# saiprasadbarke/robustmvd

Hardware: AMD Instinct MI355X
Metric: depth-maps/sec at 768x1152x4srcx256planes; warp+aggregate HBM GB/s vs roofline (higher is better)
Workload: dtype f32; 1 GPU; mvsnet (Path B) forward 768x1152, 4 source views, 256 planes, batch 1 per step (BASELINE.json configs[2]); the regulariser's two layers with 32 input channels (conv0, conv4): every fp32 operand as two range-scaled fp16 terms on fp16 MFMA, fp32 accumulation (at least as close to a float64 convolution as the fp32 matrix instruction over 1e-42..1e30: tests/test_hip_f16.py), the other nine layers and ; parallelism=1 independent replica(s), frames round-robin, no collectives

## Files before the change

### robustmvd_amd/csrc/conv3d_split.hip

```cpp
#include "mvd_common.h"
#include "split_operand.h"

#ifndef SPLIT_KO
#define SPLIT_KO 0
#endif
#ifndef SPLIT_DEPTH
#define SPLIT_DEPTH 4
#endif

namespace mvd {

typedef _Float16 h16x8 __attribute__((ext_vector_type(8)));
typedef float sf32x4 __attribute__((ext_vector_type(4)));
typedef unsigned int su32x4 __attribute__((ext_vector_type(4)));
typedef unsigned int su32x2 __attribute__((ext_vector_type(2)));
typedef _Float16 h16x2 __attribute__((ext_vector_type(2)));

constexpr int S_TH = 4, S_TW = 32, S_ROWS = S_TH + 2;
constexpr float S_LO_FACTOR = 2048.0f;
template <int CIN>
struct SplitGeom {
    static constexpr int CH8 = CIN / 8;
    static constexpr int VB = CIN * 2;
    static constexpr int KWG = CIN == 32 ? 3 : 2;
    static constexpr int NT = 9 * KWG;
    static constexpr int COLS = CIN == 32 ? S_TW + 2 : S_TW + 3;
    static constexpr int HALF_BYTES = S_ROWS * COLS * VB;
    static constexpr int PLANE_BYTES = 2 * HALF_BYTES;
    static constexpr int ITEMS = S_ROWS * COLS * CH8;
    static constexpr int NLOAD = (ITEMS + 255) / 256;
    static constexpr int NF = 4 * KWG * 2;
    static_assert(NF - 8 == 4 * NLOAD, "pass B interleaves 8 epilogue groups and 4 staging groups per item");
};

template <int CIN>
__global__ void pack_conv0_split_kernel(const float* __restrict__ w, const float* __restrict__ wscale, _Float16* __restrict__ packed, int ncb) {
    using G = SplitGeom<CIN>;
    const int e = blockIdx.x * 256 + threadIdx.x;
    if (e >= ncb * G::NT * 64 * 8) return;
    const int j = e & 7, lane = (e >> 3) & 63, t = (e >> 9) % G::NT, cb = (e >> 9) / G::NT;
    const int col = lane & 15, k = 8 * (lane >> 4) + j, cout = cb * 8 + (col & 7);
    int tap, cin;
    if constexpr (CIN == 32) { tap = t; cin = k; }
    else { const int kw = 2 * (t % 2) + k / 16; tap = kw < 3 ? (t / 2) * 3 + kw : -1; cin = k % 16; }
    const float v = tap >= 0 ? w[((size_t)cout * CIN + cin) * 27 + tap] / wscale[cout] : 0.0f;
    _Float16 hi, lo;
    split_weight(v, S_LO_FACTOR, hi, lo);
    packed[e] = col < 8 ? hi : lo;
}

struct SplitParams {
    const float* x;
    const char* wpk;
    const float* scale;
    const float* shift;
    const float* absmax;
    float* y;
    float* yamax;
    int B, D, h, w, relu;
    int cout, ncb;
    int tiles_x, tiles_y, dgroups, td, tiles_per_xcd;
};

__device__ __forceinline__ unsigned pack_h2(_Float16 a, _Float16 b) {
    const h16x2 v = {a, b};
    return __builtin_bit_cast(unsigned, v);
}

template <int CIN, bool YAMAX = false>
__global__ void __launch_bounds__(256, 2) conv0_split_kernel(SplitParams p) {
    using G = SplitGeom<CIN>;
    constexpr int S_COLS = G::COLS, S_HALF_BYTES = G::HALF_BYTES, S_PLANE_BYTES = G::PLANE_BYTES, S_ITEMS = G::ITEMS, S_NLOAD = G::NLOAD;
    constexpr int KWG = G::KWG, NT = G::NT;
    extern __shared__ __attribute__((aligned(16))) char ring[];
    const int tid = threadIdx.x, lane = tid & 63, wv = tid >> 6;
    const int D = p.D, h = p.h, w = p.w;

    const int xcd = blockIdx.x & 7;
    int j = blockIdx.x >> 3;
    const int cb = j % p.ncb; j /= p.ncb;
    const int t_in = j % p.tiles_per_xcd; j /= p.tiles_per_xcd;
    const int dg = j % p.dgroups;
    const int b = j / p.dgroups;
    const int tile = xcd * p.tiles_per_xcd + t_in;
    if (tile >= p.tiles_x * p.tiles_y) return;
    const int ty = tile / p.tiles_x, tx = tile - ty * p.tiles_x;
    const int x0 = tx * S_TW, y0 = ty * S_TH;
    const int dz0 = dg * p.td, dz1 = min(dz0 + p.td, D);

    h16x8 wf[NT];
#pragma unroll
    for (int t = 0; t < NT; ++t) wf[t] = *reinterpret_cast<const h16x8*>(p.wpk + (((size_t)cb * NT + t) * 64 + lane) * 16);

    constexpr unsigned OOB = 0x80000000u;
    unsigned gob[S_NLOAD];
    int loff[S_NLOAD];
#pragma unroll
    for (int k = 0; k < S_NLOAD; ++k) {
        const int e = tid + 256 * k;
        const int vox = e / G::CH8, ch = e % G::CH8;
        const int r = vox / S_COLS, c = vox - r * S_COLS;
        const int gy = y0 - 1 + r, gx = x0 - 1 + c;
        const bool in = e < S_ITEMS && c < S_TW + 2 && gy >= 0 && gy < h && gx >= 0 && gx < w;
        gob[k] = in ? (unsigned)(((gy * w + gx) * CIN + ch * 8) * 4) : OOB;
        if constexpr (CIN == 32) loff[k] = e < S_ITEMS ? (vox * 64 + ((ch ^ ((c >> 1) & 3)) * 16)) : -1;
        else loff[k] = e < S_ITEMS ? e * 16 : -1;
    }
    const size_t plane_f = (size_t)h * w * CIN;
    const float* xb = p.x + (size_t)b * D * plane_f;
    su32x4 pre[S_NLOAD][2];
    auto fetch = [&](int d) {
        const bool din = d >= 0 && d < D && d <= dz1;
        const __amdgpu_buffer_rsrc_t rs = __builtin_amdgcn_make_buffer_rsrc(
            const_cast<float*>(xb + (din ? (size_t)d * plane_f : 0)), 0, din ? (int)(plane_f * 4) : 0, 0x00020000);
#pragma unroll
        for (int k = 0; k < S_NLOAD; ++k) {
            pre[k][0] = __builtin_amdgcn_raw_buffer_load_b128(rs, gob[k], 0, 0);
            pre[k][1] = __builtin_amdgcn_raw_buffer_load_b128(rs, gob[k] + 16u, 0, 0);
        }
    };
    char* const dump = ring + 2 * S_PLANE_BYTES + tid * 16;
    float xs, xs_inv;
    split_xscale(p.absmax, xs, xs_inv);
    auto split2 = [xs](float a0, float a1, unsigned& hi, unsigned& lo) { mvd::split2(xs, a0, a1, hi, lo, S_LO_FACTOR); };
    auto stash = [&](int d) {
        char* slot = ring + (d & 1) * S_PLANE_BYTES;
#pragma unroll
        for (int k = 0; k < S_NLOAD; ++k) {
            su32x4 hv, lv;
#pragma unroll
            for (int q = 0; q < 4; ++q) {
                const sf32x4 v = __builtin_bit_cast(sf32x4, pre[k][q >> 1]);
                unsigned hi, lo;
                split2(v[(q & 1) * 2], v[(q & 1) * 2 + 1], hi, lo);
                hv[q] = hi; lv[q] = lo;
            }
            char* dst = loff[k] >= 0 ? slot + loff[k] : dump;
            *reinterpret_cast<su32x4*>(dst) = hv;
            *reinterpret_cast<su32x4*>(loff[k] >= 0 ? dst + S_HALF_BYTES : dst) = lv;
        }
    };

    const int col = lane & 15;
    float esc_ = p.scale[cb * 8 + (col & 7)], esh_ = p.shift[cb * 8 + (col & 7)];
    float eun_ = reinterpret_cast<const float*>(p.wpk + (size_t)p.ncb * NT * 64 * 16)[cb * 8 + (col & 7)] * xs_inv;
    const float floor_ = p.relu ? 0.f : -__builtin_inff();
    const int xh = wv & 1, rp = wv >> 1;

    int fragk[KWG];
#pragma unroll
    for (int kw = 0; kw < KWG; ++kw) {
        if constexpr (CIN == 32) {
            const int c = 16 * xh + (lane & 15) + kw;
            fragk[kw] = (2 * rp * S_COLS + c) * 64 + (((lane >> 4) ^ ((c >> 1) & 3)) * 16);
        } else {
            const int c = 16 * xh + (lane & 15) + 2 * kw;
            fragk[kw] = (2 * rp * S_COLS + c) * 32 + (lane >> 4) * 16;
        }
    }

    sf32x4 acc[3][2][2];
#pragma unroll
    for (int s = 0; s < 3; ++s)
#pragma unroll
        for (int r = 0; r < 2; ++r) { acc[s][r][0] = sf32x4{0, 0, 0, 0}; acc[s][r][1] = sf32x4{0, 0, 0, 0}; }

    unsigned yoff[2];
#pragma unroll
    for (int row = 0; row < 2; ++row) {
        const int oy = y0 + 2 * rp + row;
        yoff[row] = (col < 8 && oy < h) ? (unsigned)((((size_t)oy * w + x0 + 16 * xh + 4 * (lane >> 4)) * p.cout + cb * 8 + col) * 4) : OOB;
    }
    const int oxb = x0 + 16 * xh + 4 * (lane >> 4);
    const size_t yplane_f = (size_t)h * w * p.cout;
    const unsigned vox_b = (unsigned)p.cout * 4u;

    fetch(dz0 - 1);
    asm volatile("" : "+v"(esc_), "+v"(esh_), "+v"(eun_));
    stash(dz0 - 1);
    fetch(dz0);

    [[maybe_unused]] float amax_ = 0.f;
    for (int z = dz0 - 1; z <= dz1; ++z) {
        if (!(SPLIT_KO & 8)) __syncthreads();
        const char* slot = ring + (z & 1) * S_PLANE_BYTES;
        char* wslot = ring + ((z + 1) & 1) * S_PLANE_BYTES;
        const int din = z + 2, dout = z - 1;
        const bool in_ok = din >= 0 && din < D && din <= dz1, out_ok = dout >= dz0 && dout < dz1;
        const __amdgpu_buffer_rsrc_t rs_in = __builtin_amdgcn_make_buffer_rsrc(
            const_cast<float*>(xb + (in_ok ? (size_t)din * plane_f : 0)), 0, in_ok ? (int)(plane_f * 4) : 0, 0x00020000);
        const __amdgpu_buffer_rsrc_t rs_out = __builtin_amdgcn_make_buffer_rsrc(
            p.y + ((size_t)b * D + (out_ok ? dout : 0)) * yplane_f, 0, out_ok ? (int)(yplane_f * 4) : 0, 0x00020000);
        int ox = oxb;
        asm volatile("" : "+v"(ox));

        constexpr int NF = G::NF, NR = 2 * NF, DEPTH = SPLIT_DEPTH;
        h16x8 fr[DEPTH];
        auto rr_of = [](int ro) { return ro == 0 ? 1 : ro == 1 ? 2 : ro == 2 ? 0 : 3; };
        auto frag = [&](int i) {
            const int g = i % NF, term = g & 1, kw = (g >> 1) % KWG, rr = rr_of(g / (2 * KWG));
            if (SPLIT_KO & 32) return wf[i % NT];
            return *reinterpret_cast<const h16x8*>(slot + term * S_HALF_BYTES + fragk[kw] + rr * S_COLS * G::VB);
        };
#pragma unroll
        for (int i = 0; i < DEPTH; ++i) fr[i] = frag(i);
#pragma unroll
        for (int g = 0; g < NF; ++g) {
            const int term = g & 1, kw = (g >> 1) % KWG, rr = rr_of(g / (2 * KWG));
            const h16x8 f = fr[g % DEPTH];
#pragma unroll
            for (int row = 0; row < 2; ++row) {
                const int kh = rr - row;
                if (kh < 0 || kh > 2) continue;
                if (SPLIT_KO & 16) acc[0][row][term][0] += f[0] * wf[(6 + kh) * KWG + kw][0];
                else acc[0][row][term] = __builtin_amdgcn_mfma_f32_16x16x32_f16(f, wf[(6 + kh) * KWG + kw], acc[0][row][term], 0, 0, 0);
            }
            fr[g % DEPTH] = frag(g + DEPTH);
            __builtin_amdgcn_sched_barrier(0);
        }
        float hl = __shfl_down(acc[0][0][0][0], 8, 16);
        unsigned hq0 = 0, lq0 = 0;
#pragma unroll
        for (int g = 0; g < NF; ++g) {
            const int term = g & 1, kw = (g >> 1) % KWG, rr = rr_of(g / (2 * KWG));
            const h16x8 f = fr[(NF + g) % DEPTH];
#pragma unroll
            for (int row = 0; row < 2; ++row) {
                const int kh = rr - row;
                if (kh < 0 || kh > 2) continue;
#pragma unroll
                for (int s = 1; s < 3; ++s)
                    if (SPLIT_KO & 16) acc[s][row][term][0] += f[0] * wf[((2 - s) * 3 + kh) * KWG + kw][0];
                    else acc[s][row][term] = __builtin_amdgcn_mfma_f32_16x16x32_f16(f, wf[((2 - s) * 3 + kh) * KWG + kw], acc[s][row][term], 0, 0, 0);
            }
            if (NF + g + DEPTH < NR) fr[(NF + g) % DEPTH] = frag(NF + g + DEPTH);
            if (g < 8) {
                const int row = g >> 2, i = g & 3;
                const float cur = hl;
                if (g + 1 < 8) hl = __shfl_down(acc[0][(g + 1) >> 2][0][(g + 1) & 3], 8, 16);
                float r = __builtin_fmaf(cur + acc[0][row][1][i], 1.0f / 2048.0f, acc[0][row][0][i]);
                r = fmaxf(__builtin_fmaf(r * eun_, esc_, esh_), floor_);
                if constexpr (YAMAX)
                    if (out_ok && yoff[row] != OOB && ox + i < w) amax_ = fmaxf(amax_, finite_abs_or_zero(r));
                if (!(SPLIT_KO & 2) || r == 12345.678f)
                    __builtin_amdgcn_raw_buffer_store_b32(__float_as_uint(r), rs_out, ox + i < w ? yoff[row] + vox_b * i : OOB, 0, 0);
            } else if (!(SPLIT_KO & 4)) {
                const int k = (g - 8) >> 2, q = (g - 8) & 3;
                const sf32x4 v = __builtin_bit_cast(sf32x4, pre[k][q >> 1]);
                unsigned hq1, lq1;
                split2(v[(q & 1) * 2], v[(q & 1) * 2 + 1], hq1, lq1);
                if (q & 1) {
                    char* dst = (loff[k] >= 0 ? wslot + loff[k] : dump) + 8 * (q >> 1);
                    *reinterpret_cast<su32x2*>(dst) = su32x2{hq0, hq1};
                    *reinterpret_cast<su32x2*>(loff[k] >= 0 ? dst + S_HALF_BYTES : dst) = su32x2{lq0, lq1};
                } else {
                    hq0 = hq1; lq0 = lq1;
                }
                if (q == 3 && !(SPLIT_KO & 1)) {
                    pre[k][0] = __builtin_amdgcn_raw_buffer_load_b128(rs_in, gob[k], 0, 0);
                    pre[k][1] = __builtin_amdgcn_raw_buffer_load_b128(rs_in, gob[k] + 16u, 0, 0);
                }
            }
            __builtin_amdgcn_sched_barrier(0);
        }
#pragma unroll
        for (int r = 0; r < 2; ++r)
#pragma unroll
            for (int t = 0; t < 2; ++t) {
                acc[0][r][t] = acc[1][r][t];
                acc[1][r][t] = acc[2][r][t];
                acc[2][r][t] = sf32x4{0, 0, 0, 0};
            }
    }
    if constexpr (YAMAX) {
        for (int o = 32; o > 0; o >>= 1) amax_ = fmaxf(amax_, __shfl_xor(amax_, o));
        __syncthreads();
        float* wm = reinterpret_cast<float*>(ring);
        if (lane == 0) wm[wv] = amax_;
        __syncthreads();
        if (tid == 0) {
            amax_ = fmaxf(fmaxf(wm[0], wm[1]), fmaxf(wm[2], wm[3]));
            raise_absmax(p.yamax, amax_);
        }
    }
}

}

static bool split_shape_ok(int Cin, int Cout) { return (Cin == 32 || Cin == 16) && Cout >= 8 && Cout <= 64 && Cout % 8 == 0; }
static size_t split_frag_bytes(int Cin, int Cout) { return (size_t)(Cout / 8) * (Cin == 32 ? 27 : 18) * 64 * 16; }

template <int CIN, bool YAMAX>
static int launch_split_v(const mvd::SplitParams& p, long long nblk, hipStream_t st) {
    const size_t lds = 2 * (size_t)mvd::SplitGeom<CIN>::PLANE_BYTES + 256 * 16;
    (void)hipFuncSetAttribute((const void*)mvd::conv0_split_kernel<CIN, YAMAX>, hipFuncAttributeMaxDynamicSharedMemorySize, (int)lds);
    hipLaunchKernelGGL((mvd::conv0_split_kernel<CIN, YAMAX>), dim3((unsigned)nblk), dim3(256), lds, st, p);
    return mvd::launch_status("conv3d_split");
}
template <int CIN>
static int launch_split(const mvd::SplitParams& p, long long nblk, hipStream_t st) {
    return p.yamax ? launch_split_v<CIN, true>(p, nblk, st) : launch_split_v<CIN, false>(p, nblk, st);
}

extern "C" {

size_t mvd_conv3d_split_packed_weight_bytes(int Cin, int Cout) {
    return split_shape_ok(Cin, Cout) ? split_frag_bytes(Cin, Cout) + (size_t)Cout * sizeof(float) : 0;
}

int mvd_pack_conv3d_weights_split(const float* w, int Cin, int Cout, void* packed, mvd_stream_t stream) {
    MVD_REQUIRE(w && packed, "pack_conv3d_weights_split: NULL argument");
    MVD_REQUIRE(split_shape_ok(Cin, Cout), "pack_conv3d_weights_split: 16 or 32 input channels and 8, 16, ... 64 output channels are built (got %d -> %d)", Cin, Cout);
    const int ncb = Cout / 8;
    float* wscale = reinterpret_cast<float*>(static_cast<char*>(packed) + split_frag_bytes(Cin, Cout));
    mvd::split_wscale_launch(w, wscale, Cin, Cout, 27, false, Cout, Cout, (hipStream_t)stream);
    const unsigned nb = (unsigned)((split_frag_bytes(Cin, Cout) / 2 + 255) / 256);
    if (Cin == 32) hipLaunchKernelGGL(mvd::pack_conv0_split_kernel<32>, dim3(nb), dim3(256), 0, (hipStream_t)stream, w, wscale, (_Float16*)packed, ncb);
    else hipLaunchKernelGGL(mvd::pack_conv0_split_kernel<16>, dim3(nb), dim3(256), 0, (hipStream_t)stream, w, wscale, (_Float16*)packed, ncb);
    return mvd::launch_status("pack_conv3d_weights_split");
}

static int conv3d_split_entry(const float* x, const float* x_absmax, const void* packed_w, const float* scale, const float* shift, float* y,
                              float* y_absmax, int B, int D, int h, int w, int Cin, int Cout, int relu, mvd_stream_t stream);

int mvd_conv3d_bn_relu_f32_split(const float* x, const float* x_absmax, const void* packed_w, const float* scale, const float* shift,
                                 float* y, int B, int D, int h, int w, int Cin, int Cout, int relu, mvd_stream_t stream) {
    return conv3d_split_entry(x, x_absmax, packed_w, scale, shift, y, nullptr, B, D, h, w, Cin, Cout, relu, stream);
}

int mvd_conv3d_bn_relu_absmax_f32_split(const float* x, const float* x_absmax, const void* packed_w, const float* scale, const float* shift,
                                        float* y, float* y_absmax, int B, int D, int h, int w, int Cin, int Cout, int relu,
                                        mvd_stream_t stream) {
    MVD_REQUIRE(y_absmax, "conv3d_split_absmax: NULL argument");
    return conv3d_split_entry(x, x_absmax, packed_w, scale, shift, y, y_absmax, B, D, h, w, Cin, Cout, relu, stream);
}

static int conv3d_split_entry(const float* x, const float* x_absmax, const void* packed_w, const float* scale, const float* shift, float* y,
                              float* y_absmax, int B, int D, int h, int w, int Cin, int Cout, int relu, mvd_stream_t stream) {
    MVD_REQUIRE(x && x_absmax && packed_w && scale && shift && y, "conv3d_split: NULL argument");
    MVD_REQUIRE(split_shape_ok(Cin, Cout), "conv3d_split: 16 or 32 input channels and 8, 16, ... 64 output channels are built (got %d -> %d)", Cin, Cout);
    MVD_REQUIRE(B > 0 && D > 0 && h > 0 && w > 0, "conv3d_split: non-positive dimension");
    MVD_REQUIRE((long long)h * w * Cin * 4 < 0x7fffffffLL && (long long)h * w * Cout * 4 < 0x7fffffffLL,
                "conv3d_split: one plane exceeds the 31-bit byte-offset range");
    mvd::SplitParams p{};
    p.x = x; p.absmax = x_absmax; p.wpk = (const char*)packed_w; p.scale = scale; p.shift = shift; p.y = y; p.yamax = y_absmax;
    if (y_absmax && hipMemsetAsync(y_absmax, 0, sizeof(float), (hipStream_t)stream) != hipSuccess) return mvd::launch_status("conv3d_split: memset");
    p.B = B; p.D = D; p.h = h; p.w = w; p.relu = relu;
    p.cout = Cout; p.ncb = Cout / 8;
    p.tiles_x = (w + mvd::S_TW - 1) / mvd::S_TW;
    p.tiles_y = (h + mvd::S_TH - 1) / mvd::S_TH;
    const long long tiles = (long long)p.tiles_x * p.tiles_y;
    p.tiles_per_xcd = (int)((tiles + 7) / 8);
    int td = 32;
    while (td > 8 && tiles * B * p.ncb * ((D + td - 1) / td) < 2048) td /= 2;
    p.td = td;
    p.dgroups = (D + td - 1) / td;
    const long long nblk = 8LL * p.ncb * p.tiles_per_xcd * p.dgroups * B;
    MVD_REQUIRE(nblk <= 0x7fffffffLL, "conv3d_split: %lld workgroups exceed the grid limit", nblk);
    return Cin == 32 ? launch_split<32>(p, nblk, (hipStream_t)stream) : launch_split<16>(p, nblk, (hipStream_t)stream);
}
}
```

Baseline: 348.9 depth-maps/sec.

## Add optional 8-row tile variant and configurable staging schedule to split conv kernel

Templates the split-fp16 conv kernel on tile height, adding an 8-row, 512-thread variant that is compiled only under experiment flags and selected through an environment variable. Moves the fp32-to-fp16 split staging into a lambda that a compile-time schedule can spread across pass A and pass B groups. With the default SPLIT_SCHED=1 that schedule still places staging only in pass B, now evenly spread when fewer staging steps exist than slots. The march-depth heuristic now also counts waves per block, with a higher threshold. At TH=4 the effective threshold is unchanged, so defaults keep a 4-row tile with essentially the same behaviour.

```diff
diff --git a/robustmvd_amd/csrc/conv3d_split.hip b/robustmvd_amd/csrc/conv3d_split.hip
--- a/robustmvd_amd/csrc/conv3d_split.hip
+++ b/robustmvd_amd/csrc/conv3d_split.hip
@@ -6,6 +6,12 @@
 #endif
 #ifndef SPLIT_DEPTH
 #define SPLIT_DEPTH 4
+#endif
+#ifndef SPLIT_TH
+#define SPLIT_TH 0
+#endif
+#ifndef SPLIT_SCHED
+#define SPLIT_SCHED 1
 #endif
 
 namespace mvd {
@@ -16,10 +22,14 @@
 typedef unsigned int su32x2 __attribute__((ext_vector_type(2)));
 typedef _Float16 h16x2 __attribute__((ext_vector_type(2)));
 
-constexpr int S_TH = 4, S_TW = 32, S_ROWS = S_TH + 2;
+constexpr int S_TW = 32;
 constexpr float S_LO_FACTOR = 2048.0f;
-template <int CIN>
+template <int CIN, int TH>
 struct SplitGeom {
+    static_assert(TH == 4 || TH == 8, "the tile is 4 or 8 rows");
+    static constexpr int NW = TH;
+    static constexpr int NTHR = 64 * NW;
+    static constexpr int S_ROWS = TH + 2;
     static constexpr int CH8 = CIN / 8;
     static constexpr int VB = CIN * 2;
     static constexpr int KWG = CIN == 32 ? 3 : 2;
@@ -28,14 +38,25 @@
     static constexpr int HALF_BYTES = S_ROWS * COLS * VB;
     static constexpr int PLANE_BYTES = 2 * HALF_BYTES;
     static constexpr int ITEMS = S_ROWS * COLS * CH8;
-    static constexpr int NLOAD = (ITEMS + 255) / 256;
+    static constexpr int NLOAD = (ITEMS + NTHR - 1) / NTHR;
     static constexpr int NF = 4 * KWG * 2;
-    static_assert(NF - 8 == 4 * NLOAD, "pass B interleaves 8 epilogue groups and 4 staging groups per item");
+    static constexpr int LDS_BYTES = 2 * PLANE_BYTES + NTHR * 16;
+    static_assert(NF - 8 >= 4 * NLOAD, "pass B interleaves 8 epilogue groups and 4 staging groups per item");
+    static constexpr int stage_step(int pass, int g) {
+        constexpr int STEPS = 4 * NLOAD;
+        const bool both = SPLIT_SCHED == 3;
+        if (pass == 0 ? !both : g < 8) return -1;
+        const int SLOTS = both ? 2 * NF - 8 : NF - 8, slot = pass == 0 ? g : both ? NF + g - 8 : g - 8;
+        if (SPLIT_SCHED == 0) return slot < STEPS ? slot : -1;
+        if (SPLIT_SCHED == 2) return slot - (SLOTS - STEPS);
+        const int j = (slot * STEPS + SLOTS - 1) / SLOTS;
+        return j < STEPS && j * SLOTS / STEPS == slot ? j : -1;
+    }
 };
 
 template <int CIN>
 __global__ void pack_conv0_split_kernel(const float* __restrict__ w, const float* __restrict__ wscale, _Float16* __restrict__ packed, int ncb) {
-    using G = SplitGeom<CIN>;
+    using G = SplitGeom<CIN, 4>;
     const int e = blockIdx.x * 256 + threadIdx.x;
     if (e >= ncb * G::NT * 64 * 8) return;
     const int j = e & 7, lane = (e >> 3) & 63, t = (e >> 9) % G::NT, cb = (e >> 9) / G::NT;
@@ -67,10 +88,10 @@
     return __builtin_bit_cast(unsigned, v);
 }
 
-template <int CIN, bool YAMAX = false>
-__global__ void __launch_bounds__(256, 2) conv0_split_kernel(SplitParams p) {
-    using G = SplitGeom<CIN>;
-    constexpr int S_COLS = G::COLS, S_HALF_BYTES = G::HALF_BYTES, S_PLANE_BYTES = G::PLANE_BYTES, S_ITEMS = G::ITEMS, S_NLOAD = G::NLOAD;
+template <int CIN, int TH, bool YAMAX = false>
+__global__ void __launch_bounds__(64 * TH, TH == 4 ? 2 : 1) conv0_split_kernel(SplitParams p) {
+    using G = SplitGeom<CIN, TH>;
+    constexpr int S_TH = TH, NTHR = G::NTHR, S_COLS = G::COLS, S_HALF_BYTES = G::HALF_BYTES, S_PLANE_BYTES = G::PLANE_BYTES, S_ITEMS = G::ITEMS, S_NLOAD = G::NLOAD;
     constexpr int KWG = G::KWG, NT = G::NT;
     extern __shared__ __attribute__((aligned(16))) char ring[];
     const int tid = threadIdx.x, lane = tid & 63, wv = tid >> 6;
@@ -97,7 +118,7 @@
     int loff[S_NLOAD];
 #pragma unroll
     for (int k = 0; k < S_NLOAD; ++k) {
-        const int e = tid + 256 * k;
+        const int e = tid + NTHR * k;
         const int vox = e / G::CH8, ch = e % G::CH8;
         const int r = vox / S_COLS, c = vox - r * S_COLS;
         const int gy = y0 - 1 + r, gx = x0 - 1 + c;
@@ -204,6 +225,25 @@
         };
 #pragma unroll
         for (int i = 0; i < DEPTH; ++i) fr[i] = frag(i);
+        unsigned hq0 = 0, lq0 = 0;
+        auto stage = [&](int s) {
+            if (s < 0 || (SPLIT_KO & 4)) return;
+            const int k = s >> 2, q = s & 3;
+            const sf32x4 v = __builtin_bit_cast(sf32x4, pre[k][q >> 1]);
+            unsigned hq1, lq1;
+            split2(v[(q & 1) * 2], v[(q & 1) * 2 + 1], hq1, lq1);
+            if (q & 1) {
+                char* dst = (loff[k] >= 0 ? wslot + loff[k] : dump) + 8 * (q >> 1);
+                *reinterpret_cast<su32x2*>(dst) = su32x2{hq0, hq1};
+                *reinterpret_cast<su32x2*>(loff[k] >= 0 ? dst + S_HALF_BYTES : dst) = su32x2{lq0, lq1};
+            } else {
+                hq0 = hq1; lq0 = lq1;
+            }
+            if (q == 3 && !(SPLIT_KO & 1)) {
+                pre[k][0] = __builtin_amdgcn_raw_buffer_load_b128(rs_in, gob[k], 0, 0);
+                pre[k][1] = __builtin_amdgcn_raw_buffer_load_b128(rs_in, gob[k] + 16u, 0, 0);
+            }
+        };
 #pragma unroll
         for (int g = 0; g < NF; ++g) {
             const int term = g & 1, kw = (g >> 1) % KWG, rr = rr_of(g / (2 * KWG));
@@ -216,10 +256,10 @@
                 else acc[0][row][term] = __builtin_amdgcn_mfma_f32_16x16x32_f16(f, wf[(6 + kh) * KWG + kw], acc[0][row][term], 0, 0, 0);
             }
             fr[g % DEPTH] = frag(g + DEPTH);
+            stage(G::stage_step(0, g));
             __builtin_amdgcn_sched_barrier(0);
         }
         float hl = __shfl_down(acc[0][0][0][0], 8, 16);
-        unsigned hq0 = 0, lq0 = 0;
 #pragma unroll
         for (int g = 0; g < NF; ++g) {
             const int term = g & 1, kw = (g >> 1) % KWG, rr = rr_of(g / (2 * KWG));
@@ -244,22 +284,8 @@
                     if (out_ok && yoff[row] != OOB && ox + i < w) amax_ = fmaxf(amax_, finite_abs_or_zero(r));
                 if (!(SPLIT_KO & 2) || r == 12345.678f)
                     __builtin_amdgcn_raw_buffer_store_b32(__float_as_uint(r), rs_out, ox + i < w ? yoff[row] + vox_b * i : OOB, 0, 0);
-            } else if (!(SPLIT_KO & 4)) {
-                const int k = (g - 8) >> 2, q = (g - 8) & 3;
-                const sf32x4 v = __builtin_bit_cast(sf32x4, pre[k][q >> 1]);
-                unsigned hq1, lq1;
-                split2(v[(q & 1) * 2], v[(q & 1) * 2 + 1], hq1, lq1);
-                if (q & 1) {
-                    char* dst = (loff[k] >= 0 ? wslot + loff[k] : dump) + 8 * (q >> 1);
-                    *reinterpret_cast<su32x2*>(dst) = su32x2{hq0, hq1};
-                    *reinterpret_cast<su32x2*>(loff[k] >= 0 ? dst + S_HALF_BYTES : dst) = su32x2{lq0, lq1};
-                } else {
-                    hq0 = hq1; lq0 = lq1;
-                }
-                if (q == 3 && !(SPLIT_KO & 1)) {
-                    pre[k][0] = __builtin_amdgcn_raw_buffer_load_b128(rs_in, gob[k], 0, 0);
-                    pre[k][1] = __builtin_amdgcn_raw_buffer_load_b128(rs_in, gob[k] + 16u, 0, 0);
-                }
+            } else {
+                stage(G::stage_step(1, g));
             }
             __builtin_amdgcn_sched_barrier(0);
         }
@@ -279,7 +305,7 @@
         if (lane == 0) wm[wv] = amax_;
         __syncthreads();
         if (tid == 0) {
-            amax_ = fmaxf(fmaxf(wm[0], wm[1]), fmaxf(wm[2], wm[3]));
+            for (int i = 0; i < G::NW; ++i) amax_ = fmaxf(amax_, wm[i]);
             raise_absmax(p.yamax, amax_);
         }
     }
@@ -290,16 +316,32 @@
 static bool split_shape_ok(int Cin, int Cout) { return (Cin == 32 || Cin == 16) && Cout >= 8 && Cout <= 64 && Cout % 8 == 0; }
 static size_t split_frag_bytes(int Cin, int Cout) { return (size_t)(Cout / 8) * (Cin == 32 ? 27 : 18) * 64 * 16; }
 
-template <int CIN, bool YAMAX>
+#if defined(MVD_EXPERIMENTS) || SPLIT_TH == 8
+#define SPLIT_HAS_TILE8 1
+#else
+#define SPLIT_HAS_TILE8 0
+#endif
+static int split_tile_rows() {
+    if (SPLIT_TH) return SPLIT_TH;
+    const char* e = mvd::exp_env("MVD_K4_CONV0_TH");
+    return SPLIT_HAS_TILE8 && e && atoi(e) == 8 ? 8 : 4;
+}
+static int split_march_depth(long long tiles, int waves, int B, int ncb, int D) {
+    int td = 32;
+    while (td > 8 && tiles * B * ncb * ((D + td - 1) / td) * waves < 8192) td /= 2;
+    return td;
+}
+
+template <int CIN, int TH, bool YAMAX>
 static int launch_split_v(const mvd::SplitParams& p, long long nblk, hipStream_t st) {
-    const size_t lds = 2 * (size_t)mvd::SplitGeom<CIN>::PLANE_BYTES + 256 * 16;
-    (void)hipFuncSetAttribute((const void*)mvd::conv0_split_kernel<CIN, YAMAX>, hipFuncAttributeMaxDynamicSharedMemorySize, (int)lds);
-    hipLaunchKernelGGL((mvd::conv0_split_kernel<CIN, YAMAX>), dim3((unsigned)nblk), dim3(256), lds, st, p);
+    using G = mvd::SplitGeom<CIN, TH>;
+    (void)hipFuncSetAttribute((const void*)mvd::conv0_split_kernel<CIN, TH, YAMAX>, hipFuncAttributeMaxDynamicSharedMemorySize, G::LDS_BYTES);
+    hipLaunchKernelGGL((mvd::conv0_split_kernel<CIN, TH, YAMAX>), dim3((unsigned)nblk), dim3(G::NTHR), G::LDS_BYTES, st, p);
     return mvd::launch_status("conv3d_split");
 }
-template <int CIN>
+template <int CIN, int TH>
 static int launch_split(const mvd::SplitParams& p, long long nblk, hipStream_t st) {
-    return p.yamax ? launch_split_v<CIN, true>(p, nblk, st) : launch_split_v<CIN, false>(p, nblk, st);
+    return p.yamax ? launch_split_v<CIN, TH, true>(p, nblk, st) : launch_split_v<CIN, TH, false>(p, nblk, st);
 }
 
 extern "C" {
@@ -348,15 +390,18 @@
     p.B = B; p.D = D; p.h = h; p.w = w; p.relu = relu;
     p.cout = Cout; p.ncb = Cout / 8;
     p.tiles_x = (w + mvd::S_TW - 1) / mvd::S_TW;
-    p.tiles_y = (h + mvd::S_TH - 1) / mvd::S_TH;
+    const int th = split_tile_rows();
+    p.tiles_y = (h + th - 1) / th;
     const long long tiles = (long long)p.tiles_x * p.tiles_y;
     p.tiles_per_xcd = (int)((tiles + 7) / 8);
-    int td = 32;
-    while (td > 8 && tiles * B * p.ncb * ((D + td - 1) / td) < 2048) td /= 2;
-    p.td = td;
-    p.dgroups = (D + td - 1) / td;
+    p.td = split_march_depth(tiles, th, B, p.ncb, D);
+    p.dgroups = (D + p.td - 1) / p.td;
     const long long nblk = 8LL * p.ncb * p.tiles_per_xcd * p.dgroups * B;
     MVD_REQUIRE(nblk <= 0x7fffffffLL, "conv3d_split: %lld workgroups exceed the grid limit", nblk);
-    return Cin == 32 ? launch_split<32>(p, nblk, (hipStream_t)stream) : launch_split<16>(p, nblk, (hipStream_t)stream);
-}
-}
+    const hipStream_t st = (hipStream_t)stream;
+#if SPLIT_HAS_TILE8
+    if (th == 8) return Cin == 32 ? launch_split<32, 8>(p, nblk, st) : launch_split<16, 8>(p, nblk, st);
+#endif
+    return Cin == 32 ? launch_split<32, 4>(p, nblk, st) : launch_split<16, 4>(p, nblk, st);
+}
+}
```

Result: no change. 349.9 depth-maps/sec, median of 2 (+0.3%).
